# maxjiang93/space_time_pde

Measured on AMD Instinct MI355X. Metric: query-points/sec (fwd+PDE-residual bwd), rb2d 128^3 latent, higher is better.
Workload: dtype f32; 1 GPU; BASELINE configs[1]: latent [1,32,128,128,32], 2^20 query points, RB2 (3 transport + continuity), ImNet nf=32 softplus, L1 losses, backward to ImNet + UNet3d parameters; points=1048576, parallelism=points sharded x1, unet=UNet3d(igres=(32, 128, 128), nf=16, mf=256) fwd+bwd inside the timed step

## Files before the change

### include/stpde_hip.h

```cpp
#ifndef STPDE_HIP_H
#define STPDE_HIP_H

#ifdef __cplusplus
extern "C" {
#endif

#define STPDE_OK 0
#define STPDE_E_BADARG 1
#define STPDE_E_UNSUPPORTED 2
#define STPDE_E_LAUNCH 3

#define STPDE_ACT_TANH 0
#define STPDE_ACT_RELU 1
#define STPDE_ACT_SOFTPLUS 2
#define STPDE_ACT_ELU 3
#define STPDE_ACT_SWISH 4
#define STPDE_ACT_LEAKYRELU 5

#define STPDE_XT 3
#define STPDE_PBAR_SLOTS 64

typedef struct {
  int S1;
  int S2;
// ... 27 lines not shown
                     float* coef, int* cell, float* cw , void* stream);

typedef struct {
  int ntiles, KT, MT, first_hidden;
  stpde_jet_cfg cfg;
  int mfma_bf16;
  int packed;
  int det;
} stpde_layer_desc;
int stpde_jet_layer_fwd(const stpde_layer_desc* d, const float* in_pre, const float* X, const float* Wh_pack,
                        const float* Ws_pack, const float* tanc, const float* W0s_pack, const float* tanc0,
                        float* out_pre, const float* cw ,
                        const void* Wh_pack_bf16, float* z0, void* stream);

int stpde_jet_tail_fwd(const stpde_jet_cfg* cfg, int ntiles, int nf16, const float* in_pre2, const float* X,
                       const float* const* Wh_pack, const float* const* Ws_pack, const float* const* tanc,
                       float* const* out_pre, const float* cw, void* stream);

int stpde_jet_tail_fwd_p(const stpde_jet_cfg* cfg, int ntiles, int nf16, const float* in_pre2, const float* X,
                         const float* const* Wh_pack, const float* const* Ws_pack, const float* const* tanc,
                         float* const* out_pre, const float* cw, int packed, const void* const* Wh16_pack, void* stream);

int stpde_jet_tail_bwd(const stpde_jet_cfg* cfg, int ntiles, int nf16, const float* abar5, const float* const* WhT_pack,
                       const float* const* pre, float* const* abar_out, const float* cw, float* act_param_bar,
                       void* stream);

int stpde_jet_tail_bwd_p(const stpde_jet_cfg* cfg, int ntiles, int nf16, const float* abar5, const float* const* WhT_pack,
                         const float* const* pre, float* const* abar_out, const float* cw, float* act_param_bar, int packed,
                         const void* const* WhT16_pack, void* stream);

int stpde_jet_layer_bwd(const stpde_layer_desc* d, const float* abar_out, const float* WhT_pack, float* in_pre,
                        const float* X, const float* W0s_pack, const float* tanc0, float* abar0, const float* cw,
                        float* act_param_bar, const void* WhT_pack_bf16 ,
                        float* abar0_tan, const float* z0, void* stream);

int stpde_jet_layer_bwd_to(const stpde_layer_desc* d, const float* abar_out, const float* WhT_pack, const float* in_pre,
                           float* abar_in, const float* cw, float* act_param_bar, const void* WhT_pack_bf16, void* stream);

int stpde_jet_wgrad(const stpde_layer_desc* d, int SP, const float* abar_out, const float* in_pre, const float* X,
                    const float* tanc0, float* dW_aug, const float* cw, void* stream);

int stpde_jet_fc1_bwd_supported(const stpde_layer_desc* d);
int stpde_jet_fc1_bwd(const stpde_layer_desc* d, const float* abar1, const void* WhT_pack_bf16, const float* z0,
                      const float* tanc0, const float* cw, const float* X, float* abar0, float* abar0_tan, float* dW_aug,
                      float* act_param_bar, void* stream);

int stpde_lig_reduce_fwd(const stpde_jet_cfg* cfg, int S_mlp, int P, int n_out, const float* out_pre,
                         const float* coef, float* jets, long ldp, void* stream);
int stpde_lig_reduce_bwd(const stpde_jet_cfg* cfg, int S_mlp, int P, int n_out, const float* jets_bar, long ldp,
                         const float* coef, float* abar_out, void* stream);

int stpde_jet_tan0_reduce(int ntiles, int MT, const float* abar0_tan, float* dW_aug, int ldw, int det ,
                          void* stream);

typedef struct {
  int ntiles, nlayers, C, n1, n2;
  int MT[8];
  int SP[8];
  int packed[8];
  int S[8];
} stpde_xbar_desc;
int stpde_lig_xbar_scatter(const stpde_xbar_desc* d, const float* const* abar, const float* const* WsL_pack,
                           const int* cell, float* dlatent, void* stream);
int stpde_lig_xbar_rows(const stpde_xbar_desc* d, const float* const* abar, const float* const* WsL_pack,
                        float* xrows, void* stream);
int stpde_lig_dlatent_reduce(int B, int n0, int n1, int n2, int C, const float* xrows, const int* perm,
                             const int* start, float* dlatent, void* stream);

typedef struct {
  int nlayers;
  int cin, cout, nf16;
  int KT[8], MT[8];
  const float* Wh[8];
  const float* WhT[8];
  const float* Ws[8];
  const float* WsL[8];
  const float* tanc[8];
  const void* Wh16[8];
  const void* WhT16[8];
  int mfma_bf16;
  int packed_mask;
  long dw_off[8];
} stpde_imnet_plan;
typedef struct {
  float* X;
  float* XR;
  float* coef;
  float* cw;
  int* cell;
  float* pre[8];
  float* abar2x;
  float* abar3x;
  float* tan0;
  float* abar0;
  float* abar1x;
  float* abar0x;
  float* xrows;
  int* perm;
  int* start;
  void* sort_tmp;
  unsigned long sort_tmp_bytes;
  float* abar4x;
} stpde_lig_workspace;
#define STPDE_F_STASH 1
#define STPDE_F_VALUE_TILES 2
#define STPDE_F_FUSED_TAIL 4
// ... 246 lines not shown
```

### space_time_pde_amd/_lib.py

```python
import ctypes as C
import os
import subprocess
import threading

_HERE = os.path.dirname(os.path.abspath(__file__))
_CSRC = os.path.join(_HERE, "csrc")
LIB_PATH = os.environ.get("STPDE_LIB") or os.path.join(_HERE, "libstpde_hip.so")
_SOURCES = ["jet_layer.hip", "jet_layer_s00.hip", "jet_layer_s03.hip", "jet_layer_s30.hip", "jet_layer_s31.hip", "jet_layer_s32.hip", "jet_layer_s34.hip", "jet_layer_s36.hip", "jet_tail.hip", "jet_wgrad.hip", "jet_wgrad_s00.hip", "jet_wgrad_s30.hip", "jet_wgrad_s31.hip", "jet_wgrad_s32.hip", "jet_wgrad_s34.hip", "jet_wgrad_s36.hip", "jet_fc1_bwd.hip", "lig_gather_reduce.hip", "lig_pipeline.hip", "interp_nd.hip", "conv3d.hip", "conv3d_fused.hip", "optim.hip", "residual.hip", "bn.hip", "resample.hip", "sampler.hip", "sampler_median.hip", "api.cpp"]
_HIPFLAGS = ["--offload-arch=gfx950", "-O3", "-std=c++17", "-fPIC", "-ffp-contract=off", "-munsafe-fp-atomics",
             "--offload-compress"]

ABI_VERSION = 316

ACT_CODES = {"tanh": 0, "relu": 1, "softplus": 2, "elu": 3, "swish": 4, "leakyrelu": 5}
PBAR_SLOTS = 64
XT = 3


class JetCfg(C.Structure):
    _fields_ = [("S1", C.c_int), ("S2", C.c_int), ("pair0", C.c_int * 6), ("pair1", C.c_int * 6),
                ("act", C.c_int), ("act_param", C.c_float), ("combo", C.c_int), ("alpha", C.c_float * 6)]


class GatherDesc(C.Structure):
# ... 167 lines not shown
        objs.append(o)
        ostamp = o + ".srchash"
        owant = _source_hash([s] + _includes(s))
        if not force and os.path.exists(o) and os.path.exists(ostamp) and open(ostamp).read().strip() == owant:
            continue
        flags = _HIPFLAGS if s.endswith(".hip") else ["-O3", "-std=c++17", "-fPIC"]
        cmd = ["hipcc"] + flags + ["-c", s, "-o", o]
        if verbose:
            print(" ".join(cmd))
        procs.append((cmd, ostamp, owant, subprocess.Popen(cmd, stdout=subprocess.PIPE, stderr=subprocess.STDOUT)))
    for cmd, ostamp, owant, p in procs:
        out, _ = p.communicate()
        if p.returncode != 0:
            raise RuntimeError("hipcc failed: %s\n%s" % (" ".join(cmd), out.decode()))
        with open(ostamp, "w") as f:
            f.write(owant)
    cmd = ["hipcc", "--offload-arch=gfx950", "--offload-compress", "-shared", "-fPIC", "-o", LIB_PATH] + objs
    r = subprocess.run(cmd, stdout=subprocess.PIPE, stderr=subprocess.STDOUT)
    if r.returncode != 0:
        raise RuntimeError("link failed: %s\n%s" % (" ".join(cmd), r.stdout.decode()))
    with open(stamp, "w") as f:
        f.write(want)
    return LIB_PATH


_lib = None
_lock = threading.Lock()
_VP = C.c_void_p

_SIGNATURES = {
    "stpde_version": ([], C.c_int),
    "stpde_last_error": ([C.c_char_p, C.c_ulong], C.c_int),
    "stpde_tune": ([C.c_char_p, C.c_int], C.c_int),
    "stpde_trace_enable": ([C.c_int], C.c_int),
    "stpde_trace_read": ([C.c_char_p, C.c_ulong], C.c_long),
    "stpde_lig_gather": ([C.POINTER(GatherDesc), _VP, _VP, _VP, _VP, _VP, _VP, _VP, _VP], C.c_int),
    "stpde_lig_gather_nd": ([C.POINTER(GatherNdDesc), _VP, _VP, _VP, _VP, _VP], C.c_int),
    "stpde_lig_reduce_nd_fwd": ([C.c_int, C.c_int, C.c_int, C.c_int, _VP, _VP, _VP, C.c_long, _VP], C.c_int),
    "stpde_lig_reduce_nd_bwd": ([C.c_int, C.c_int, C.c_int, C.c_int, _VP, C.c_long, _VP, _VP, _VP], C.c_int),
    "stpde_lig_cell_nd": ([C.POINTER(GatherNdDesc), _VP, _VP, _VP], C.c_int),
    "stpde_lig_dlatent_reduce_nd": ([C.c_int, C.c_int, C.POINTER(C.c_int), C.c_int, _VP, _VP, _VP, _VP, _VP], C.c_int),
    "stpde_jet_layer_fwd": ([C.POINTER(LayerDesc)] + [_VP] * 12, C.c_int),
    "stpde_jet_layer_bwd": ([C.POINTER(LayerDesc)] + [_VP] * 13, C.c_int),
    "stpde_jet_layer_bwd_to": ([C.POINTER(LayerDesc)] + [_VP] * 8, C.c_int),
    "stpde_jet_tail_fwd": ([C.POINTER(JetCfg), C.c_int, C.c_int, _VP, _VP, C.POINTER(_VP), C.POINTER(_VP), C.POINTER(_VP),
                            C.POINTER(_VP), _VP, _VP], C.c_int),
    "stpde_jet_tail_bwd": ([C.POINTER(JetCfg), C.c_int, C.c_int, _VP, C.POINTER(_VP), C.POINTER(_VP), C.POINTER(_VP), _VP,
                            _VP, _VP], C.c_int),
    "stpde_jet_tail_fwd_p": ([C.POINTER(JetCfg), C.c_int, C.c_int, _VP, _VP, C.POINTER(_VP), C.POINTER(_VP), C.POINTER(_VP),
                              C.POINTER(_VP), _VP, C.c_int, C.POINTER(_VP), _VP], C.c_int),
    "stpde_jet_tail_bwd_p": ([C.POINTER(JetCfg), C.c_int, C.c_int, _VP, C.POINTER(_VP), C.POINTER(_VP), C.POINTER(_VP), _VP,
                              _VP, C.c_int, C.POINTER(_VP), _VP], C.c_int),
    "stpde_jet_tan0_reduce": ([C.c_int, C.c_int, _VP, _VP, C.c_int, C.c_int, _VP], C.c_int),
    "stpde_jet_wgrad": ([C.POINTER(LayerDesc), C.c_int] + [_VP] * 7, C.c_int),
    "stpde_jet_fc1_bwd_supported": ([C.POINTER(LayerDesc)], C.c_int),
    "stpde_jet_fc1_bwd": ([C.POINTER(LayerDesc)] + [_VP] * 11, C.c_int),
    "stpde_lig_reduce_fwd": ([C.POINTER(JetCfg), C.c_int, C.c_int, C.c_int, _VP, _VP, _VP, C.c_long, _VP], C.c_int),
    "stpde_lig_reduce_bwd": ([C.POINTER(JetCfg), C.c_int, C.c_int, C.c_int, _VP, C.c_long, _VP, _VP, _VP], C.c_int),
    "stpde_lig_xbar_scatter": ([C.POINTER(XbarDesc), C.POINTER(_VP), C.POINTER(_VP), _VP, _VP, _VP], C.c_int),
    "stpde_lig_xbar_rows": ([C.POINTER(XbarDesc), C.POINTER(_VP), C.POINTER(_VP), _VP, _VP], C.c_int),
    "stpde_lig_dlatent_reduce": ([C.c_int] * 5 + [_VP] * 5, C.c_int),
    "stpde_lig_imnet_jet_fwd": ([C.POINTER(ImNetPlanDesc), C.POINTER(JetCfg), C.POINTER(JetCfg), C.POINTER(GatherDesc), _VP,
                                 _VP, C.POINTER(LigWorkspace), _VP, C.c_long, C.c_int, _VP], C.c_int),
    "stpde_lig_imnet_jet_bwd": ([C.POINTER(ImNetPlanDesc), C.POINTER(JetCfg), C.POINTER(JetCfg), C.POINTER(JetCfg),
                                 C.POINTER(GatherDesc), C.POINTER(LigWorkspace), _VP, C.c_long, _VP, _VP, _VP, C.c_int, _VP],
                                C.c_int),
    "stpde_lig_sort_tmp_bytes": ([C.c_int, C.c_long], C.c_ulong),
    "stpde_lig_cell_sort": ([C.c_int, C.c_long, _VP, _VP, _VP, _VP, C.c_ulong, _VP], C.c_int),
    "stpde_interp_fwd": ([C.POINTER(InterpDesc)] + [_VP] * 7, C.c_int),
    "stpde_interp_bwd_grid": ([C.POINTER(InterpDesc)] + [_VP] * 5, C.c_int),
    "stpde_conv3d_fwd": ([C.POINTER(Conv3dDesc)] + [_VP] * 5, C.c_int),
    "stpde_conv3d_wgrad": ([C.POINTER(Conv3dDesc)] + [_VP] * 4, C.c_int),
    "stpde_conv3d_wgrad_bias": ([C.POINTER(Conv3dDesc)] + [_VP] * 5, C.c_int),
    "stpde_conv3d_fused": ([C.POINTER(Conv3dFusedArgs), C.POINTER(C.c_int), _VP], C.c_int),
    "stpde_conv3d_wgrad_onload": ([C.POINTER(Conv3dDesc)] + [_VP] * 8, C.c_int),
    "stpde_residual_fwd": ([_VP, C.c_int, C.c_int, C.c_int, C.c_int, _VP, C.c_long, C.c_long, _VP, _VP, _VP], C.c_int),
    "stpde_residual_bwd": ([_VP, C.c_int, C.c_int, C.c_int, C.c_int, _VP, C.c_long, C.c_long, _VP, _VP, _VP, _VP],
                           C.c_int),
    "stpde_resample3d": ([C.POINTER(ResampleDesc), C.c_int, _VP, _VP, _VP, _VP], C.c_int),
    "stpde_det_finalize": ([_VP, C.c_long, _VP, _VP], C.c_int),
    "stpde_bn_fwd": ([C.POINTER(BnDesc)] + [_VP] * 10, C.c_int),
    "stpde_bn_bwd": ([C.POINTER(BnDesc)] + [_VP] * 11, C.c_int),
    "stpde_loss_sum": ([C.c_int, C.c_long, _VP, _VP, _VP, _VP], C.c_int),
    "stpde_loss_grad": ([C.c_int, C.c_long, _VP, _VP, _VP, _VP, _VP], C.c_int),
    "stpde_clip_adam": ([C.POINTER(AdamDesc)] + [_VP] * 5, C.c_int),
    "stpde_clip_adam_multi": ([C.POINTER(AdamDesc), _VP, _VP, C.c_int, C.c_int, _VP], C.c_int),
    "stpde_opt_advance": ([C.POINTER(OptDesc), _VP, _VP], C.c_int),
    "stpde_clip_adam_dev": ([C.POINTER(AdamDesc)] + [_VP] * 6, C.c_int),
    "stpde_clip_adam_multi_dev": ([C.POINTER(AdamDesc), _VP, _VP, _VP, C.c_int, C.c_int, _VP], C.c_int),
    "stpde_clip_sgd": ([C.POINTER(SgdDesc)] + [_VP] * 5, C.c_int),
    "stpde_clip_sgd_multi": ([C.POINTER(SgdDesc), _VP, _VP, _VP, C.c_int, C.c_int, _VP], C.c_int),
    "stpde_sampler_draw": ([C.POINTER(SamplerDesc)] + [_VP] * 4, C.c_int),
    "stpde_sampler_produce": ([C.POINTER(SamplerDesc)] + [_VP] * 10, C.c_int),
    "stpde_sampler_filter": ([C.POINTER(SamplerFilterDesc)] + [_VP] * 9, C.c_int),
    "stpde_sampler_produce_filtered": ([C.POINTER(SamplerDesc)] + [_VP] * 8, C.c_int),
    "stpde_sampler_median": ([C.POINTER(SamplerFilterDesc)] + [_VP] * 5, C.c_int),
}


def exported_symbols():
    return sorted(_SIGNATURES)


def register_signatures(sigs):
    _SIGNATURES.update(sigs)

# ... 123 lines not shown
```

### space_time_pde_amd/csrc/common.h

```cpp
#pragma once
#include <hip/hip_runtime.h>

#include "../../include/stpde_hip.h"

typedef float f32x4 __attribute__((ext_vector_type(4)));

#define XT STPDE_XT
__host__ __device__ constexpr int x_live(int xt) { return xt == XT - 1 ? 1 : 4; }

__device__ __forceinline__ f32x4 ld4x(const float* p, int xt) {
  if (xt == XT - 1) return f32x4{p[0], 0.f, 0.f, 0.f};
  return *reinterpret_cast<const f32x4*>(p);
}

__device__ __forceinline__ f32x4 mfma4(float a, float b, f32x4 c) {
  return __builtin_amdgcn_mfma_f32_16x16x4f32(a, b, c, 0, 0, 0);
}

typedef __bf16 bf16x4 __attribute__((ext_vector_type(4)));
typedef __bf16 bf16x8 __attribute__((ext_vector_type(8)));
__device__ __forceinline__ bf16x4 to_bf4(f32x4 v) {
  bf16x4 r;
#pragma unroll
  for (int i = 0; i < 4; ++i) r[i] = (__bf16)v[i];
// ... 211 lines not shown
__device__ __forceinline__ f32x2 sel3(int d, f32x2 a0, f32x2 a1, f32x2 a2) { return d == 0 ? a0 : (d == 1 ? a1 : a2); }

template <int ACT>
__device__ __forceinline__ ActDT<f32x2> act_eval2_t(float prm, f32x2 a) {
  STPDE_JET_FMA
  ActDT<f32x2> r;
  if (ACT == STPDE_ACT_SOFTPLUS) {
    const f32x2 t = f32x2{-fabsf(a.x), -fabsf(a.y)} * 1.44269504088896341f;
    const f32x2 e = f32x2{__builtin_amdgcn_exp2f(t.x), __builtin_amdgcn_exp2f(t.y)};
    const f32x2 u = e + 1.f;
    const f32x2 inv = f32x2{fast_rcp(u.x), fast_rcp(u.y)};
    const f32x2 einv = e * inv;
    const f32x2 s = sel2(a.x >= 0.f, a.y >= 0.f, inv, einv);
    const f32x2 q = einv * inv;
    const bool b0 = a.x > 20.f, b1 = a.y > 20.f;
    const f32x2 lbig = f32x2{__builtin_amdgcn_logf(u.x), __builtin_amdgcn_logf(u.y)} * 0.693147180559945309f;
    const f32x2 lsmall = e * (1.f - e * (0.5f - e * 0.33333334f));
    const f32x2 l1p = sel2(e.x < 9.765625e-4f, e.y < 9.765625e-4f, lsmall, lbig);
    r.s0 = f32x2{fmaxf(a.x, 0.f), fmaxf(a.y, 0.f)} + l1p;
    const f32x2 one = f32x2{1.f, 1.f}, zero = f32x2{0.f, 0.f};
    r.s1 = sel2(b0, b1, one, s);
    r.s2 = sel2(b0, b1, zero, q);
    r.s3 = sel2(b0, b1, zero, q * (1.f - 2.f * s));
  } else {
    const ActD x = act_eval_t<ACT>(prm, a.x), y = act_eval_t<ACT>(prm, a.y);
    r.s0 = f32x2{x.s0, y.s0};
    r.s1 = f32x2{x.s1, y.s1};
    r.s2 = f32x2{x.s2, y.s2};
    r.s3 = f32x2{x.s3, y.s3};
  }
  return r;
}
template <int ACT>
__device__ __forceinline__ ActDT<f32x2> act_eval2(int act, float prm, f32x2 a) {
  if (ACT >= 0) return act_eval2_t<(ACT >= 0 ? ACT : 0)>(prm, a);
  const ActD x = act_eval<ACT>(act, prm, a.x), y = act_eval<ACT>(act, prm, a.y);
  ActDT<f32x2> r;
  r.s0 = f32x2{x.s0, y.s0};
  r.s1 = f32x2{x.s1, y.s1};
  r.s2 = f32x2{x.s2, y.s2};
  r.s3 = f32x2{x.s3, y.s3};
  return r;
}
template <int ACT>
__device__ __forceinline__ ActDT<float> act_eval_w(int act, float prm, float a) {
  const ActD s = act_eval<ACT>(act, prm, a);
  return ActDT<float>{s.s0, s.s1, s.s2, s.s3};
}
template <int ACT>
__device__ __forceinline__ ActDT<f32x2> act_eval_w(int act, float prm, f32x2 a) {
  return act_eval2<ACT>(act, prm, a);
}

template <int S1, int S2, int ACT, class T>
__device__ __forceinline__ void act_jet_fwd_w(const stpde_jet_cfg& cfg, const T* pre, T* h, const float* cq) {
  STPDE_JET_FMA
  const ActDT<T> s = act_eval_w<ACT>(cfg.act, cfg.act_param, pre[0]);
  h[0] = s.s0;
  if (S1 == 3) {
    const T a0 = pre[1], a1 = pre[2], a2 = pre[3];
    h[1] = s.s1 * a0;
    h[2] = s.s1 * a1;
    h[3] = s.s1 * a2;
    if (S2 == 1) {
      const T q = a0 * (cq[0] * a0 + cq[1] * a1 + cq[2] * a2) + a1 * (cq[3] * a1 + cq[4] * a2) + cq[5] * a2 * a2;
      h[4] = s.s2 * q + s.s1 * pre[4];
      return;
    }
#pragma unroll
    for (int p = 0; p < S2; ++p) {
      const T u = sel3(cfg.pair0[p], a0, a1, a2), v = sel3(cfg.pair1[p], a0, a1, a2);
      h[4 + p] = s.s2 * u * v + s.s1 * pre[4 + p];
    }
  }
}
template <int S1, int S2, int ACT>
__device__ __forceinline__ void act_jet_fwd(const stpde_jet_cfg& cfg, const f32x4* pre, f32x4* h,
                                            const float* cq = nullptr) {
  STPDE_JET_FMA
  constexpr int S = 1 + S1 + S2;
  if (S1 == 0 && S2 > 0) {
#pragma unroll
    for (int st = 0; st < 1 + S2; ++st) {
#if STPDE_JET_PACKED
      h[st].lo = act_eval_w<ACT>(cfg.act, cfg.act_param, (f32x2)pre[st].lo).s0;
      h[st].hi = act_eval_w<ACT>(cfg.act, cfg.act_param, (f32x2)pre[st].hi).s0;
#else
#pragma unroll
      for (int r = 0; r < 4; ++r) h[st][r] = act_eval<ACT>(cfg.act, cfg.act_param, pre[st][r]).s0;
#endif
    }
    return;
  }
#if STPDE_JET_PACKED
#pragma unroll
  for (int half = 0; half < 2; ++half) {
    f32x2 p2[S], h2[S];
#pragma unroll
    for (int st = 0; st < S; ++st) p2[st] = half ? (f32x2)pre[st].hi : (f32x2)pre[st].lo;
    act_jet_fwd_w<S1, S2, ACT, f32x2>(cfg, p2, h2, cq);
#pragma unroll
    for (int st = 0; st < S; ++st) {
      if (half) h[st].hi = h2[st];
      else h[st].lo = h2[st];
    }
  }
#else
#pragma unroll
  for (int r = 0; r < 4; ++r) {
    float p1[S], h1[S];
#pragma unroll
    for (int st = 0; st < S; ++st) p1[st] = pre[st][r];
    act_jet_fwd_w<S1, S2, ACT, float>(cfg, p1, h1, cq);
#pragma unroll
    for (int st = 0; st < S; ++st) h[st][r] = h1[st];
  }
#endif
}

template <int S1, int S2, int ACT, class T>
__device__ __forceinline__ void act_jet_adj_w(const stpde_jet_cfg& cfg, const T* pre, const T* hbar, T* abar, const float* cq) {
  STPDE_JET_FMA
  const ActDT<T> s = act_eval_w<ACT>(cfg.act, cfg.act_param, pre[0]);
  T ab = s.s1 * hbar[0];
  if (S1 == 3) {
    const T a0 = pre[1], a1 = pre[2], a2 = pre[3];
    T d0 = s.s1 * hbar[1], d1 = s.s1 * hbar[2], d2 = s.s1 * hbar[3];
    ab += s.s2 * (a0 * hbar[1] + a1 * hbar[2] + a2 * hbar[3]);
    if (S2 == 1) {
      const T hb = hbar[4];
      const T q = a0 * (cq[0] * a0 + cq[1] * a1 + cq[2] * a2) + a1 * (cq[3] * a1 + cq[4] * a2) + cq[5] * a2 * a2;
      ab += (s.s3 * q + s.s2 * pre[4]) * hb;
      const T t = s.s2 * hb;
      d0 += t * (2.f * cq[0] * a0 + cq[1] * a1 + cq[2] * a2);
      d1 += t * (cq[1] * a0 + 2.f * cq[3] * a1 + cq[4] * a2);
      d2 += t * (cq[2] * a0 + cq[4] * a1 + 2.f * cq[5] * a2);
      abar[4] = s.s1 * hb;
    }
#pragma unroll
    for (int p = 0; p < (S2 == 1 ? 0 : S2); ++p) {
      const int e0 = cfg.pair0[p], e1 = cfg.pair1[p];
      const T u = sel3(e0, a0, a1, a2), v = sel3(e1, a0, a1, a2);
      const T hb = hbar[4 + p];
      ab += (s.s3 * u * v + s.s2 * pre[4 + p]) * hb;
      const T t0 = s.s2 * v * hb;
      const T t1 = s.s2 * u * hb;
      const T z = t0 * 0.f;
      d0 += (e0 == 0 ? t0 : z) + (e1 == 0 ? t1 : z);
      d1 += (e0 == 1 ? t0 : z) + (e1 == 1 ? t1 : z);
      d2 += (e0 == 2 ? t0 : z) + (e1 == 2 ? t1 : z);
      abar[4 + p] = s.s1 * hb;
    }
    abar[1] = d0;
// ... 254 lines not shown
```

### space_time_pde_amd/csrc/jet_layer.hip

```cpp
#include "jet_layer_impl.h"

static int dispatch_streams(const LayerArgs& a, int mode, hipStream_t stream) {
  const int S1 = a.cfg.S1, S2 = a.cfg.S2;
  if (S1 == 0 && S2 == 0) return stpde_layer_launch_0_0(a, mode, stream);
  if (S1 == 0 && S2 == 3) return stpde_layer_launch_0_3(a, mode, stream);
  if (S1 == 3 && S2 == 0) return stpde_layer_launch_3_0(a, mode, stream);
  if (S1 == 3 && S2 == 1 && a.cfg.combo && a.cw) return stpde_layer_launch_3_1(a, mode, stream);
  if (S1 == 3 && S2 == 2) return stpde_layer_launch_3_2(a, mode, stream);
  if (S1 == 3 && S2 == 4) return stpde_layer_launch_3_4(a, mode, stream);
  if (S1 == 3 && S2 == 6) return stpde_layer_launch_3_6(a, mode, stream);
  stpde_set_error("stream configuration S1=%d S2=%d not compiled (supported: (0,0) (0,3 = four value tiles, forward only) (3,0) (3,1 combined, needs cw) (3,2) (3,4) (3,6))", S1, S2);
  return STPDE_E_UNSUPPORTED;
}

static int check_cfg(const stpde_layer_desc* d) {
  if (!d || d->ntiles <= 0 || d->MT <= 0 || d->KT < 0) {
    stpde_set_error("layer desc: bad sizes");
    return STPDE_E_BADARG;
  }
  if (d->cfg.act < 0 || d->cfg.act > 5) {
    stpde_set_error("layer desc: unknown activation %d", d->cfg.act);
    return STPDE_E_BADARG;
  }
  for (int p = 0; p < d->cfg.S2 && p < 6; ++p)
// ... 67 lines not shown
    return STPDE_E_BADARG;
  }
  return layer_bwd(d, abar_out, WhT_pack, in_pre, abar_in, nullptr, nullptr, nullptr, nullptr, cw, act_param_bar,
                   WhT_pack_bf16, nullptr, nullptr, stream);
}

static int layer_bwd(const stpde_layer_desc* d, const float* abar_out, const float* WhT_pack, const float* in_pre,
                     float* abar_in, const float* X, const float* W0s_pack, const float* tanc0, float* abar0,
                     const float* cw, float* act_param_bar, const void* WhT_pack_bf16, float* abar0_tan, const float* z0,
                     void* stream) {
  int rc = check_cfg(d);
  if (rc) return rc;
  LayerArgs a{};
  a.Bin = abar_out;
  a.Wp = WhT_pack;
  a.X = X;
  a.W0s = W0s_pack;
  a.tanc0 = tanc0;
  a.cw = cw;
  a.pbar = act_param_bar;
  a.Wp16 = d->mfma_bf16 ? WhT_pack_bf16 : nullptr;
  a.nsplit = d->mfma_bf16 == 3 ? 3 : 1;
  a.KT = d->MT;
  a.MT = d->KT;
  a.ntiles = d->ntiles;
  a.cfg = d->cfg;
  a.pk = ((d->packed & 4) ? 1 : 0) | ((d->packed & 2) ? 2 : 0) | ((d->packed & 1) ? 4 : 0);
  if (!abar_out || !WhT_pack || d->KT <= 0) {
    stpde_set_error("jet_layer_bwd: null pointer / no hidden input");
    return STPDE_E_BADARG;
  }
  if (d->first_hidden) {
    if (!z0 || !abar0 || (d->cfg.S1 && !tanc0)) {
      stpde_set_error("jet_layer_bwd: first_hidden needs z0/tanc0/abar0");
      return STPDE_E_BADARG;
    }
    if (z0 == abar0 && d->cfg.S1 && !abar0_tan) {
      stpde_set_error("jet_layer_bwd: z0 may alias abar0 only when abar0 holds the value stream alone");
      return STPDE_E_BADARG;
    }
    a.Out = abar0;
    a.Tan0 = abar0_tan;
    a.Z0 = const_cast<float*>(z0);
    return dispatch_streams(a, 3, (hipStream_t)stream);
  }
  if (!in_pre || !abar_in) {
    stpde_set_error("jet_layer_bwd: null in_pre");
    return STPDE_E_BADARG;
  }
  a.Out = abar_in;
  a.Pre = in_pre;
  return dispatch_streams(a, 2, (hipStream_t)stream);
}
```

### space_time_pde_amd/csrc/jet_layer_impl.h

```cpp
#pragma once
#include <cstdlib>

#include "common.h"

enum { PRO_NONE = 0, PRO_ACT = 1, PRO_L0 = 2 };
enum { EPI_FWD = 0, EPI_ADJ = 1, EPI_ADJ_L0 = 2 };
#ifndef STPDE_ABLATE
#define STPDE_ABLATE 0
#endif

#ifndef STPDE_STAMP
#define STPDE_STAMP 0
#endif
#ifndef STPDE_FWD2_OCC3
#define STPDE_FWD2_OCC3 1
#endif
#ifndef STPDE_FWD2_OCC_N
#define STPDE_FWD2_OCC_N 3
#endif
#ifndef STPDE_EARLY_L0
#define STPDE_EARLY_L0 1
#endif
#ifndef STPDE_EPI_PF
#define STPDE_EPI_PF 1
// ... 16 lines not shown
#ifndef STPDE_X3_Z0P
#define STPDE_X3_Z0P 0
#endif
#ifndef STPDE_SKIP_FIRST_BAR
#define STPDE_SKIP_FIRST_BAR 1
#endif
#if STPDE_STAMP
#define STPDE_STAMP_B0 8192
static __device__ unsigned long long g_stamp[256 * 8 * 16];
#define STAMP(i)                                                                                          \
  do {                                                                                                    \
    if (blockIdx.x >= STPDE_STAMP_B0 && blockIdx.x < STPDE_STAMP_B0 + 256 && (threadIdx.x & 63) == 0)     \
      g_stamp[((blockIdx.x - STPDE_STAMP_B0) * 8 + (threadIdx.x >> 6)) * 16 + (i)] = __builtin_readcyclecounter(); \
  } while (0)
#else
#define STAMP(i)
#endif

struct LayerArgs {
  const float* Bin;
  const float* Wp;
  const float* X;
  const float* W0s;
  const float* tanc0;
  const float* Wsp;
  const float* tanc;
  float* Out;
  const float* Pre;
  const float* cw;
  const void* Wp16;
  int nsplit;
  float* pbar;
  float* Tan0;
  float* Z0;
  int KT, MT, ntiles;
  int split;
  int pk;
  stpde_jet_cfg cfg;
};

__device__ __forceinline__ f32x4 layer0_block(const float* W0s, int nblk, int blk, int lo, const f32x4* xb) {
  f32x4 part[XT];
#pragma unroll
  for (int xt = 0; xt < XT; ++xt) {
    f32x4 w = ld4x(W0s + ((size_t)xt * nblk + blk) * 256 + lo, xt);
    f32x4 c = f32x4{0.f, 0.f, 0.f, 0.f};
#pragma unroll
    for (int r = 0; r < x_live(xt); ++r) c = mfma4(w[r], xb[xt][r], c);
    part[xt] = c;
  }
  return (part[0] + part[1]) + part[2];
}

template <int S1, int S2, int EPI, int ACT, int PKM = 0>
__device__ __forceinline__ void layer_epilogue(const LayerArgs& a, int tile, int mt, int MT, int lane, f32x4* accm,
                                               const f32x4 (*xbv)[XT], const float* cq, float& pacc,
                                               const f32x4* z0pre = nullptr, const f32x4* prepf = nullptr,
                                               const f32x4* wspf = nullptr, const f32x4* tcpf = nullptr) {
  constexpr int S = 1 + S1 + S2;
  constexpr bool VT = S1 == 0 && S2 > 0;
  const int lo = lane * 4;
  f32x4 (&acc)[1][S] = *reinterpret_cast<f32x4 (*)[1][S]>(accm);
  constexpr int mi = 0;
    if (EPI == EPI_FWD) {
#pragma unroll
      for (int xt = 0; xt < XT; ++xt) {
        f32x4 w = wspf ? wspf[xt] : ld4x(a.Wsp + ((size_t)xt * MT + mt) * 256 + lo, xt);
#pragma unroll
        for (int sv = 0; sv < (VT ? S : 1); ++sv)
#pragma unroll
          for (int r = 0; r < x_live(xt); ++r) acc[mi][sv] = mfma4(w[r], xbv[sv][xt][r], acc[mi][sv]);
      }
      if (S1 == 3) {
#pragma unroll
        for (int d = 0; d < 3; ++d) acc[mi][1 + d] += tcpf ? tcpf[d] : ld4(a.tanc + ((size_t)d * MT + mt) * 256 + lo);
      }
#pragma unroll
      for (int st = 0; st < S; ++st) st_blk(a.Out, (PKM & 2) ? 1 : 0, tile, S, MT, st, mt, lane, acc[mi][st]);
    } else {
      f32x4 pre[S], ab[S];
      if (EPI == EPI_ADJ) {
#pragma unroll
        for (int st = 0; st < S; ++st)
          pre[st] = prepf ? prepf[st] : ld_blk(a.Pre, (PKM & 4) ? 1 : 0, tile, S, MT, st, mt, lane);
      } else {
        pre[0] = z0pre ? *z0pre : ld4(a.Z0 + ((size_t)tile * MT + mt) * 256 + lo);
        if (S1 == 3) {
#pragma unroll
          for (int d = 0; d < 3; ++d) pre[1 + d] = tcpf ? tcpf[d] : ld4(a.tanc0 + ((size_t)d * MT + mt) * 256 + lo);
#pragma unroll
          for (int p = 0; p < S2; ++p) pre[4 + p] = f32x4{0.f, 0.f, 0.f, 0.f};
        }
      }
      act_jet_adj<S1, S2, ACT>(a.cfg, pre, acc[mi], ab, cq);
      if ((ACT == STPDE_ACT_SWISH || (ACT < 0 && a.cfg.act == STPDE_ACT_SWISH)) && a.pbar)
        pacc += swish_beta_adj<S1, S2>(a.cfg, pre, acc[mi], cq);
      constexpr int SO = (EPI == EPI_ADJ) ? S : 1 + S1;
      if (EPI == EPI_ADJ_L0 && S1 == 3 && a.Tan0) {
        st_blk(a.Out, (PKM & 2) ? 2 : 0, tile, 1, MT, 0, mt, lane, ab[0]);
        f32x4 ts[3];
#pragma unroll
        for (int d = 0; d < 3; ++d) ts[d] = row_sum16x4(ab[1 + d]);
        if ((lane & 15) == 15) {
          float* tp = a.Tan0 + ((size_t)tile * MT + mt) * 48 + 4 * (lane >> 4);
#pragma unroll
          for (int d = 0; d < 3; ++d) st4(tp + 16 * d, ts[d]);
        }
      } else {
#pragma unroll
        for (int st = 0; st < SO; ++st) st_blk(a.Out, (PKM & 2) ? 2 : 0, tile, SO, MT, st, mt, lane, ab[st]);
      }
    }
}

template <int EPI, int ACT>
__device__ __forceinline__ void flush_pbar(const LayerArgs& a, float pacc, int lane) {
  if (EPI != EPI_FWD && (ACT == STPDE_ACT_SWISH || (ACT < 0 && a.cfg.act == STPDE_ACT_SWISH)) && a.pbar) {
    const float v = wave_sum(pacc);
    if (lane == 0) atomicAdd(a.pbar + (blockIdx.x % STPDE_PBAR_SLOTS), v);
  }
}

template <int S1, int S2, int MC, int PRO, int EPI, int ACT, bool GUARD>
__global__ __launch_bounds__(256) void k_layer(LayerArgs a) {
  constexpr int S = 1 + S1 + S2;
  const int lane = threadIdx.x & 63;
  const int tile = blockIdx.x * 4 + (threadIdx.x >> 6);
  if (tile >= a.ntiles) return;
  const int KT = a.KT, MT = a.MT;
  const int lo = lane * 4;
  float cq[6];
  load_cq<S2>(a.cw, tile * 2 + ((lane & 15) >> 3), cq);
  float pacc = 0.f;

  constexpr bool VT = S1 == 0 && S2 > 0;
  constexpr int NX = VT ? S : 1;
  f32x4 xb[NX][XT];
  if (PRO == PRO_L0 || EPI == EPI_FWD) {
#pragma unroll
    for (int sv = 0; sv < NX; ++sv)
#pragma unroll
      for (int xt = 0; xt < XT; ++xt) xb[sv][xt] = ld4x(a.X + (((size_t)tile * NX + sv) * XT + xt) * 256 + lo, xt);
  }
  const auto z0r = opt_store_rsrc(a.Z0 ? a.Z0 + (size_t)tile * KT * 256 : nullptr, (unsigned)KT * 1024u);

  for (int mt0 = 0; mt0 < MT; mt0 += MC) {
  f32x4 acc[MC][S];
#pragma unroll
  for (int mi = 0; mi < MC; ++mi)
#pragma unroll
    for (int st = 0; st < S; ++st) acc[mi][st] = f32x4{0.f, 0.f, 0.f, 0.f};
  const float* wp = a.Wp + (size_t)mt0 * 256 + lo;

  auto load_raw = [&](int kt, f32x4* raw) {
    if (PRO == PRO_L0) {
#pragma unroll
      for (int sv = 0; sv < NX; ++sv) raw[sv] = layer0_block(a.W0s, KT, kt, lo, xb[sv]);
      if (!VT) opt_st4(z0r, kt * 1024 + lane * 16, raw[0]);
      if (S1 == 3) {
#pragma unroll
// ... 14 lines not shown
    }
  };

  if (KT > 0) {
    f32x4 Bc[S], wc[MC];
    {
      f32x4 raw[S];
      load_raw(0, raw);
      if (PRO == PRO_NONE) {
#pragma unroll
        for (int st = 0; st < S; ++st) Bc[st] = raw[st];
      } else {
        act_jet_fwd<S1, S2, ACT>(a.cfg, raw, Bc, cq);
      }
      load_w(0, wc);
    }
    for (int kt = 0; kt < KT; ++kt) {
      const int kn = kt + 1 < KT ? kt + 1 : kt;
      f32x4 rawn[S], wn[MC];
      load_raw(kn, rawn);
      load_w(kn, wn);
#pragma unroll
      for (int mi = 0; mi < MC; ++mi)
#pragma unroll
        for (int r = 0; r < 4; ++r)
#pragma unroll
          for (int st = 0; st < S; ++st) acc[mi][st] = mfma4(wc[mi][r], Bc[st][r], acc[mi][st]);
      if (PRO == PRO_NONE) {
#pragma unroll
        for (int st = 0; st < S; ++st) Bc[st] = rawn[st];
      } else {
        act_jet_fwd<S1, S2, ACT>(a.cfg, rawn, Bc, cq);
      }
#pragma unroll
      for (int mi = 0; mi < MC; ++mi) wc[mi] = wn[mi];
    }
  }

#pragma unroll
  for (int mi = 0; mi < MC; ++mi) {
    const int mt = mt0 + mi;
    if (GUARD && mt >= MT) continue;
    layer_epilogue<S1, S2, EPI, ACT>(a, tile, mt, MT, lane, acc[mi], xb, cq, pacc);
  }
  }
  flush_pbar<EPI, ACT>(a, pacc, lane);
}


template <int S1, int S2, int MCg, int PRO, int EPI, int ACT, int NW, bool BF = false, int PK = 1, bool WRING = false,
          int SPL = 1, int PKM = 0>
__global__ __launch_bounds__(64 * NW, ((!BF || SPL == 1) && PRO == PRO_ACT && EPI == EPI_FWD && MCg == 2 && NW == 4 && !WRING && S1 + S2 <= 4 && STPDE_FWD2_OCC3) ? STPDE_FWD2_OCC_N : 2) void k_layer_coop(LayerArgs a) {
  constexpr int S = 1 + S1 + S2, GK = NW * PK;
  static_assert(!WRING || (!BF && GK == 4), "the weight ring is written for 4 k-tiles per group, fp32");
  static_assert(SPL == 1 || (BF && SPL == 3), "operand splitting is a bf16-pipe mode");
  constexpr int BMODE = (PKM & 1) ? (EPI == EPI_FWD ? 1 : 2) : 0;
  __shared__ __attribute__((aligned(16))) float hb[2][GK][S][BF ? 128 * SPL : 256];
  const int lane = threadIdx.x & 63;
  const int wv = threadIdx.x >> 6;
  const int KT = a.KT, MT = a.MT;
  const int lo = lane * 4;
  STAMP(0);
  int tile = blockIdx.x, pass0 = 0, pstep = 1;
  if (a.split > 0) {
    const int L = blockIdx.x, xcd = L & 7, slot = L >> 3;
    pass0 = slot % a.split;
    pstep = a.split;
    tile = (slot / a.split) * 8 + xcd;
    if (tile >= a.ntiles) return;
  }
  float cq[6];
  load_cq<S2>(a.cw, tile * 2 + ((lane & 15) >> 3), cq);
  float pacc = 0.f;

  constexpr bool VT = S1 == 0 && S2 > 0;
  constexpr int NX = VT ? S : 1;
  f32x4 xb[NX][XT];
  if (PRO == PRO_L0 || EPI == EPI_FWD) {
#pragma unroll
    for (int sv = 0; sv < NX; ++sv)
#pragma unroll
      for (int xt = 0; xt < XT; ++xt) xb[sv][xt] = ld4x(a.X + (((size_t)tile * NX + sv) * XT + xt) * 256 + lo, xt);
  }
  const auto z0r = opt_store_rsrc(a.Z0 ? a.Z0 + (size_t)tile * KT * 256 : nullptr, (unsigned)KT * 1024u);

  auto produce = [&](int kt, int buf, int slot) {
    f32x4 raw[S], B[S];
    if (PRO == PRO_L0) {
#pragma unroll
      for (int sv = 0; sv < NX; ++sv) raw[sv] = layer0_block(a.W0s, KT, kt, lo, xb[sv]);
      if (!VT) opt_st4(z0r, kt * 1024 + lane * 16, raw[0]);
      if (S1 == 3) {
#pragma unroll
        for (int d = 0; d < 3; ++d) raw[1 + d] = ld4(a.tanc0 + ((size_t)d * KT + kt) * 256 + lo);
#pragma unroll
        for (int p = 0; p < S2; ++p) raw[4 + p] = f32x4{0.f, 0.f, 0.f, 0.f};
      }
    } else {
#pragma unroll
      for (int st = 0; st < S; ++st) raw[st] = ld_blk(a.Bin, BMODE, tile, S, KT, st, kt, lane);
    }
    if (PRO == PRO_NONE || STPDE_ABLATE == 1) {
#pragma unroll
      for (int st = 0; st < S; ++st) B[st] = raw[st];
    } else {
      act_jet_fwd<S1, S2, ACT>(a.cfg, raw, B, cq);
    }
#pragma unroll
    for (int st = 0; st < S; ++st) {
      if constexpr (BF) {
        f32x4 v = B[st];
#pragma unroll
        for (int t = 0; t < SPL; ++t) {
          const bf16x4 h = to_bf4(v);
          *reinterpret_cast<bf16x4*>(&hb[buf][slot][st][128 * t + lane * 2]) = h;
          if (t + 1 < SPL) v -= bf4_to_f32(h);
        }
      } else {
        st4(&hb[buf][slot][st][lo], B[st]);
      }
    }
  };
  auto store_block = [&](const f32x4* B, int buf, int slot) {
#pragma unroll
    for (int st = 0; st < S; ++st) {
      if constexpr (BF) {
        f32x4 v = B[st];
#pragma unroll
        for (int t = 0; t < SPL; ++t) {
          const bf16x4 h = to_bf4(v);
          *reinterpret_cast<bf16x4*>(&hb[buf][slot][st][128 * t + lane * 2]) = h;
          if (t + 1 < SPL) v -= bf4_to_f32(h);
        }
      } else {
        st4(&hb[buf][slot][st][lo], B[st]);
      }
    }
  };
  auto produce_group = [&](int g, int buf) {
#pragma unroll
    for (int k = 0; k < PK; ++k) produce(GK * g + NW * k + wv, buf, NW * k + wv);
  };

  const int ngroups = KT / GK;
  bool first_pass = true;
  for (int mt0 = (pass0 * NW + wv) * MCg; mt0 < MT; mt0 += pstep * NW * MCg) {
    f32x4 acc[MCg][S];
#pragma unroll
    for (int mi = 0; mi < MCg; ++mi)
#pragma unroll
      for (int st = 0; st < S; ++st) acc[mi][st] = f32x4{0.f, 0.f, 0.f, 0.f};
    constexpr bool Z0P = EPI == EPI_ADJ_L0 && (SPL == 1 || STPDE_X3_Z0P);
    f32x4 z0p[Z0P ? MCg : 1];
    if constexpr (Z0P) {
#pragma unroll
      for (int mi = 0; mi < MCg; ++mi) z0p[mi] = ld4(a.Z0 + ((size_t)tile * MT + mt0 + mi) * 256 + lo);
    }
    const float* wp = a.Wp + (size_t)mt0 * 256 + lo;
    f32x4 wr[WRING ? 4 : 1][MCg];
    if constexpr (WRING) {
#pragma unroll
      for (int q = 0; q < 3; ++q)
#pragma unroll
        for (int mi = 0; mi < MCg; ++mi) wr[q][mi] = ld4(wp + ((size_t)q * MT + mi) * 256);
    }
    if (!STPDE_SKIP_FIRST_BAR || !first_pass) __syncthreads();
    first_pass = false;
    STAMP(1);
    produce_group(0, 0);
    STAMP(2);
    __syncthreads();
    STAMP(3);
    for (int gi = 0; gi < ngroups; ++gi) {
      const int buf = gi & 1;
      const int gnext = gi + 1 < ngroups ? gi + 1 : gi;
      constexpr bool EARLY = PRO == PRO_NONE && (SPL == 1 || STPDE_X3_EARLY);
      constexpr bool EARLY0 = PRO == PRO_L0 && !VT && STPDE_EARLY_L0;
      f32x4 rawn[EARLY ? PK : 1][S];
      if constexpr (EARLY) {
#pragma unroll
        for (int k = 0; k < PK; ++k)
#pragma unroll
          for (int st = 0; st < S; ++st)
            rawn[k][st] = ld_blk(a.Bin, BMODE, tile, S, KT, st, GK * gnext + NW * k + wv, lane);
      }
      f32x4 w0n[EARLY0 ? PK : 1][XT], tcn[EARLY0 ? PK : 1][3];
      if constexpr (EARLY0) {
#pragma unroll
        for (int k = 0; k < PK; ++k) {
          const int kt = GK * gnext + NW * k + wv;
#pragma unroll
          for (int xt = 0; xt < XT; ++xt) w0n[k][xt] = ld4x(a.W0s + ((size_t)xt * KT + kt) * 256 + lo, xt);
          if (S1 == 3) {
#pragma unroll
            for (int d = 0; d < 3; ++d) tcn[k][d] = ld4(a.tanc0 + ((size_t)d * KT + kt) * 256 + lo);
          }
        }
// ... 72 lines not shown
          const int ktn = STPDE_ABLATE == 3 ? (q & 1) : (kt + 3 < KT ? kt + 3 : KT - 1);
          f32x4 B[S];
#pragma unroll
          for (int st = 0; st < S; ++st) B[st] = ld4(&hb[buf][q][st][lo]);
#pragma unroll
          for (int mi = 0; mi < MCg; ++mi)
#pragma unroll
            for (int r = 0; r < 4; ++r)
#pragma unroll
              for (int st = 0; st < S; ++st) acc[mi][st] = mfma4(wr[q][mi][r], B[st][r], acc[mi][st]);
#pragma unroll
          for (int mi = 0; mi < MCg; ++mi) wr[(q + 3) & 3][mi] = ld4(wp + ((size_t)ktn * MT + mi) * 256);
        }
      } else {
#pragma unroll
      for (int q = 0; q < GK; ++q) {
        const int kt = GK * gi + q;
        f32x4 B[S], w[MCg];
#pragma unroll
        for (int st = 0; st < S; ++st) B[st] = ld4(&hb[buf][q][st][lo]);
#pragma unroll
        for (int mi = 0; mi < MCg; ++mi) w[mi] = ld4(wp + ((size_t)kt * MT + mi) * 256);
#pragma unroll
        for (int mi = 0; mi < MCg; ++mi)
#pragma unroll
          for (int r = 0; r < 4; ++r)
#pragma unroll
            for (int st = 0; st < S; ++st) acc[mi][st] = mfma4(w[mi][r], B[st][r], acc[mi][st]);
      }
      }
      if constexpr (EARLY) {
#pragma unroll
        for (int k = 0; k < PK; ++k) store_block(rawn[k], buf ^ 1, NW * k + wv);
      } else if constexpr (EARLY0) {
#pragma unroll
        for (int k = 0; k < PK; ++k) {
          const int kt = GK * gnext + NW * k + wv;
          f32x4 raw[S], B[S], part[XT];
#pragma unroll
          for (int xt = 0; xt < XT; ++xt) {
            f32x4 c = f32x4{0.f, 0.f, 0.f, 0.f};
#pragma unroll
            for (int r = 0; r < x_live(xt); ++r) c = mfma4(w0n[k][xt][r], xb[0][xt][r], c);
            part[xt] = c;
          }
          raw[0] = (part[0] + part[1]) + part[2];
          opt_st4(z0r, kt * 1024 + lane * 16, raw[0]);
          if (S1 == 3) {
#pragma unroll
            for (int d = 0; d < 3; ++d) raw[1 + d] = tcn[k][d];
#pragma unroll
            for (int p = 0; p < S2; ++p) raw[4 + p] = f32x4{0.f, 0.f, 0.f, 0.f};
          }
          act_jet_fwd<S1, S2, ACT>(a.cfg, raw, B, cq);
          store_block(B, buf ^ 1, NW * k + wv);
        }
      } else {
        if (STPDE_ABLATE != 5) produce_group(gnext, buf ^ 1);
      }
      if (gi < 8) STAMP(4 + gi);
      if (STPDE_ABLATE != 2) __syncthreads();
    }
    STAMP(12);
    if (STPDE_ABLATE == 4) {
      f32x4 sum = f32x4{0.f, 0.f, 0.f, 0.f};
#pragma unroll
      for (int mi = 0; mi < MCg; ++mi)
#pragma unroll
        for (int st = 0; st < S; ++st) sum += acc[mi][st];
      if (sum[0] == 12345.678f) st4(a.Out + lo, sum);
      continue;
    }
    constexpr bool EPF = EPI == EPI_ADJ && (!BF || (SPL == 1 && STPDE_EPI_PF_BF)) && MCg > 1 && STPDE_EPI_PF;
    if constexpr (EPF) {
      constexpr int PMD = (PKM & 4) ? 1 : 0;
      constexpr int PFD = STPDE_EPI_PF_DEPTH < 1 ? 1 : (STPDE_EPI_PF_DEPTH > MCg ? MCg : STPDE_EPI_PF_DEPTH);
      f32x4 pr[MCg][S];
#pragma unroll
      for (int mi = 0; mi < PFD; ++mi)
#pragma unroll
        for (int st = 0; st < S; ++st) pr[mi][st] = ld_blk(a.Pre, PMD, tile, S, MT, st, mt0 + mi, lane);
#pragma unroll
      for (int mi = 0; mi < MCg; ++mi) {
        if (mi + PFD < MCg) {
#pragma unroll
          for (int st = 0; st < S; ++st) pr[mi + PFD][st] = ld_blk(a.Pre, PMD, tile, S, MT, st, mt0 + mi + PFD, lane);
        }
        __builtin_amdgcn_sched_barrier(0);
        layer_epilogue<S1, S2, EPI, ACT, PKM>(a, tile, mt0 + mi, MT, lane, acc[mi], xb, cq, pacc, nullptr, pr[mi]);
      }
    } else if constexpr (EPI == EPI_ADJ_L0 && S1 == 3 && S <= 5 && (STPDE_EPI_OPF & 1) && (SPL == 1 || (STPDE_EPI_OPF & 4))) {
      if constexpr (SPL == 1) {
        f32x4 z0l[MCg], tcl[MCg][3];
#pragma unroll
        for (int mi = 0; mi < MCg; ++mi) {
          z0l[mi] = Z0P ? z0p[Z0P ? mi : 0] : ld4(a.Z0 + ((size_t)tile * MT + mt0 + mi) * 256 + lo);
#pragma unroll
          for (int d = 0; d < 3; ++d) tcl[mi][d] = ld4(a.tanc0 + ((size_t)d * MT + mt0 + mi) * 256 + lo);
        }
        __builtin_amdgcn_sched_barrier(0);
#pragma unroll
        for (int mi = 0; mi < MCg; ++mi)
          layer_epilogue<S1, S2, EPI, ACT, PKM>(a, tile, mt0 + mi, MT, lane, acc[mi], xb, cq, pacc, &z0l[mi], nullptr, nullptr,
                                                  tcl[mi]);
      } else {
        f32x4 zc, zn, tcc[3], tcn2[3];
        auto fetch = [&](int mt, f32x4& z, f32x4* t) {
// ... 189 lines not shown
```

Before: 2.497 million query-points/s.

## Use packed-FP32 jet quadratic, DPP row-sum fold, and scalar wave index

```diff
diff --git a/include/stpde_hip.h b/include/stpde_hip.h
--- a/include/stpde_hip.h
+++ b/include/stpde_hip.h
@@ -103,6 +103,8 @@
 
 int stpde_jet_tan0_reduce(int ntiles, int MT, const float* abar0_tan, float* dW_aug, int ldw, int det ,
                           void* stream);
+
+int stpde_jet_rowsum_probe(int ntiles, const float* in, float* out, void* stream);
 
 typedef struct {
   int ntiles, nlayers, C, n1, n2;
diff --git a/space_time_pde_amd/_lib.py b/space_time_pde_amd/_lib.py
--- a/space_time_pde_amd/_lib.py
+++ b/space_time_pde_amd/_lib.py
@@ -243,6 +243,7 @@
     "stpde_jet_tail_bwd_p": ([C.POINTER(JetCfg), C.c_int, C.c_int, _VP, C.POINTER(_VP), C.POINTER(_VP), C.POINTER(_VP), _VP,
                               _VP, C.c_int, C.POINTER(_VP), _VP], C.c_int),
     "stpde_jet_tan0_reduce": ([C.c_int, C.c_int, _VP, _VP, C.c_int, C.c_int, _VP], C.c_int),
+    "stpde_jet_rowsum_probe": ([C.c_int, _VP, _VP, _VP], C.c_int),
     "stpde_jet_wgrad": ([C.POINTER(LayerDesc), C.c_int] + [_VP] * 7, C.c_int),
     "stpde_jet_fc1_bwd_supported": ([C.POINTER(LayerDesc)], C.c_int),
     "stpde_jet_fc1_bwd": ([C.POINTER(LayerDesc)] + [_VP] * 11, C.c_int),
diff --git a/space_time_pde_amd/csrc/common.h b/space_time_pde_amd/csrc/common.h
--- a/space_time_pde_amd/csrc/common.h
+++ b/space_time_pde_amd/csrc/common.h
@@ -287,7 +287,34 @@
   return act_eval2<ACT>(act, prm, a);
 }
 
-template <int S1, int S2, int ACT, class T>
+__device__ __forceinline__ f32x2 pk_mul(f32x2 a, f32x2 b) {
+  f32x2 r;
+  asm("v_pk_mul_f32 %0, %1, %2" : "=v"(r) : "v"(a), "v"(b));
+  return r;
+}
+__device__ __forceinline__ f32x2 pk_fma(f32x2 a, f32x2 b, f32x2 c) {
+  f32x2 r;
+  asm("v_pk_fma_f32 %0, %1, %2, %3" : "=v"(r) : "v"(a), "v"(b), "v"(c));
+  return r;
+}
+
+template <bool W, class T>
+__device__ __forceinline__ T jet_q(T a0, T a1, T a2, const float* cq) {
+  STPDE_JET_FMA
+  return a0 * (cq[0] * a0 + cq[1] * a1 + cq[2] * a2) + a1 * (cq[3] * a1 + cq[4] * a2) + cq[5] * a2 * a2;
+}
+template <>
+__device__ __forceinline__ f32x2 jet_q<true, f32x2>(f32x2 a0, f32x2 a1, f32x2 a2, const float* cq) {
+  const f32x2 c0 = f32x2{cq[0], cq[0]}, c1 = f32x2{cq[1], cq[1]}, c2 = f32x2{cq[2], cq[2]};
+  const f32x2 c3 = f32x2{cq[3], cq[3]}, c4 = f32x2{cq[4], cq[4]}, c5 = f32x2{cq[5], cq[5]};
+  f32x2 i0 = pk_fma(c0, a0, pk_mul(c1, a1));
+  const f32x2 i1 = pk_fma(c3, a1, pk_mul(c4, a2));
+  i0 = pk_fma(c2, a2, i0);
+  const f32x2 q = pk_fma(a0, i0, pk_mul(a1, i1));
+  return pk_fma(a2, pk_mul(c5, a2), q);
+}
+
+template <int S1, int S2, int ACT, class T, bool W = false>
 __device__ __forceinline__ void act_jet_fwd_w(const stpde_jet_cfg& cfg, const T* pre, T* h, const float* cq) {
   STPDE_JET_FMA
   const ActDT<T> s = act_eval_w<ACT>(cfg.act, cfg.act_param, pre[0]);
@@ -298,7 +325,7 @@
     h[2] = s.s1 * a1;
     h[3] = s.s1 * a2;
     if (S2 == 1) {
-      const T q = a0 * (cq[0] * a0 + cq[1] * a1 + cq[2] * a2) + a1 * (cq[3] * a1 + cq[4] * a2) + cq[5] * a2 * a2;
+      const T q = jet_q<W, T>(a0, a1, a2, cq);
       h[4] = s.s2 * q + s.s1 * pre[4];
       return;
     }
@@ -309,7 +336,7 @@
     }
   }
 }
-template <int S1, int S2, int ACT>
+template <int S1, int S2, int ACT, bool W = false>
 __device__ __forceinline__ void act_jet_fwd(const stpde_jet_cfg& cfg, const f32x4* pre, f32x4* h,
                                             const float* cq = nullptr) {
   STPDE_JET_FMA
@@ -333,7 +360,7 @@
     f32x2 p2[S], h2[S];
 #pragma unroll
     for (int st = 0; st < S; ++st) p2[st] = half ? (f32x2)pre[st].hi : (f32x2)pre[st].lo;
-    act_jet_fwd_w<S1, S2, ACT, f32x2>(cfg, p2, h2, cq);
+    act_jet_fwd_w<S1, S2, ACT, f32x2, W>(cfg, p2, h2, cq);
 #pragma unroll
     for (int st = 0; st < S; ++st) {
       if (half) h[st].hi = h2[st];
diff --git a/space_time_pde_amd/csrc/jet_layer.hip b/space_time_pde_amd/csrc/jet_layer.hip
--- a/space_time_pde_amd/csrc/jet_layer.hip
+++ b/space_time_pde_amd/csrc/jet_layer.hip
@@ -143,3 +143,24 @@
   a.Pre = in_pre;
   return dispatch_streams(a, 2, (hipStream_t)stream);
 }
+
+__global__ __launch_bounds__(256) void k_rowsum_probe(const float* in, float* out, int ntiles) {
+  const int lane = threadIdx.x & 63;
+  const int tile = blockIdx.x * 4 + (threadIdx.x >> 6);
+  if (tile >= ntiles) return;
+  f32x4 v[3];
+#pragma unroll
+  for (int d = 0; d < 3; ++d)
+#pragma unroll
+    for (int j = 0; j < 4; ++j) v[d][j] = in[((size_t)tile * 12 + 4 * d + j) * 64 + lane];
+  store_tan_rowsums(out + (size_t)tile * 48, lane, v);
+}
+
+extern "C" int stpde_jet_rowsum_probe(int ntiles, const float* in, float* out, void* stream) {
+  if (ntiles <= 0 || !in || !out) {
+    stpde_set_error("jet_rowsum_probe: bad arguments");
+    return STPDE_E_BADARG;
+  }
+  STPDE_LAUNCH(k_rowsum_probe, dim3((ntiles + 3) / 4), dim3(256), 0, (hipStream_t)stream, in, out, ntiles);
+  return stpde_check_launch("k_rowsum_probe");
+}
diff --git a/space_time_pde_amd/csrc/jet_layer_impl.h b/space_time_pde_amd/csrc/jet_layer_impl.h
--- a/space_time_pde_amd/csrc/jet_layer_impl.h
+++ b/space_time_pde_amd/csrc/jet_layer_impl.h
@@ -92,6 +92,62 @@
   return (part[0] + part[1]) + part[2];
 }
 
+__device__ __forceinline__ void row_sum16_fold12(const f32x4* v, float* e) {
+  float r0 = v[0][0], r1 = v[0][1], r2 = v[0][2], r3 = v[0][3], r4 = v[1][0], r5 = v[1][1], r6 = v[1][2], r7 = v[1][3];
+  float r8 = v[2][0], r9 = v[2][1], r10 = v[2][2], r11 = v[2][3], t0, t1, t2;
+  const unsigned long long even = 0x5555555555555555ull, low2 = 0x3333333333333333ull;
+  asm volatile(
+      "s_nop 1\n\t"
+      "v_cndmask_b32_e64 %12, %1, %0, %15\n\t"
+      "v_cndmask_b32_e64 %13, %3, %2, %15\n\t"
+      "v_cndmask_b32_e64 %14, %5, %4, %15\n\t"
+      "v_cndmask_b32_e64 %0, %0, %1, %15\n\t"
+      "v_cndmask_b32_e64 %2, %2, %3, %15\n\t"
+      "v_cndmask_b32_e64 %4, %4, %5, %15\n\t"
+      "v_add_f32_dpp %1, %0, %12 quad_perm:[1,0,3,2] row_mask:0xf bank_mask:0xf\n\t"
+      "v_add_f32_dpp %3, %2, %13 quad_perm:[1,0,3,2] row_mask:0xf bank_mask:0xf\n\t"
+      "v_add_f32_dpp %5, %4, %14 quad_perm:[1,0,3,2] row_mask:0xf bank_mask:0xf\n\t"
+      "v_cndmask_b32_e64 %12, %7, %6, %15\n\t"
+      "v_cndmask_b32_e64 %13, %9, %8, %15\n\t"
+      "v_cndmask_b32_e64 %14, %11, %10, %15\n\t"
+      "v_cndmask_b32_e64 %6, %6, %7, %15\n\t"
+      "v_cndmask_b32_e64 %8, %8, %9, %15\n\t"
+      "v_cndmask_b32_e64 %10, %10, %11, %15\n\t"
+      "v_add_f32_dpp %7, %6, %12 quad_perm:[1,0,3,2] row_mask:0xf bank_mask:0xf\n\t"
+      "v_add_f32_dpp %9, %8, %13 quad_perm:[1,0,3,2] row_mask:0xf bank_mask:0xf\n\t"
+      "v_add_f32_dpp %11, %10, %14 quad_perm:[1,0,3,2] row_mask:0xf bank_mask:0xf\n\t"
+      "v_cndmask_b32_e64 %12, %3, %1, %16\n\t"
+      "v_cndmask_b32_e64 %13, %7, %5, %16\n\t"
+      "v_cndmask_b32_e64 %14, %11, %9, %16\n\t"
+      "v_cndmask_b32_e64 %1, %1, %3, %16\n\t"
+      "v_cndmask_b32_e64 %5, %5, %7, %16\n\t"
+      "v_cndmask_b32_e64 %9, %9, %11, %16\n\t"
+      "v_add_f32_dpp %3, %1, %12 quad_perm:[2,3,0,1] row_mask:0xf bank_mask:0xf\n\t"
+      "v_add_f32_dpp %7, %5, %13 quad_perm:[2,3,0,1] row_mask:0xf bank_mask:0xf\n\t"
+      "v_add_f32_dpp %11, %9, %14 quad_perm:[2,3,0,1] row_mask:0xf bank_mask:0xf\n\t"
+      "v_add_f32_dpp %3, %3, %3 row_shr:4 row_mask:0xf bank_mask:0xf bound_ctrl:1\n\t"
+      "v_add_f32_dpp %7, %7, %7 row_shr:4 row_mask:0xf bank_mask:0xf bound_ctrl:1\n\t"
+      "v_add_f32_dpp %11, %11, %11 row_shr:4 row_mask:0xf bank_mask:0xf bound_ctrl:1\n\t"
+      "v_add_f32_dpp %3, %3, %3 row_shr:8 row_mask:0xf bank_mask:0xf bound_ctrl:1\n\t"
+      "v_add_f32_dpp %7, %7, %7 row_shr:8 row_mask:0xf bank_mask:0xf bound_ctrl:1\n\t"
+      "v_add_f32_dpp %11, %11, %11 row_shr:8 row_mask:0xf bank_mask:0xf bound_ctrl:1"
+      : "+v"(r0), "+v"(r1), "+v"(r2), "+v"(r3), "+v"(r4), "+v"(r5), "+v"(r6), "+v"(r7), "+v"(r8), "+v"(r9), "+v"(r10),
+        "+v"(r11), "=&v"(t0), "=&v"(t1), "=&v"(t2)
+      : "s"(even), "s"(low2));
+  e[0] = r3;
+  e[1] = r7;
+  e[2] = r11;
+}
+__device__ __forceinline__ void store_tan_rowsums(float* tan, int lane, const f32x4* ab_tan) {
+  float e[3];
+  row_sum16_fold12(ab_tan, e);
+  if ((lane & 15) >= 12) {
+    float* tp = tan + 4 * (lane >> 4) + (lane & 3);
+#pragma unroll
+    for (int d = 0; d < 3; ++d) tp[16 * d] = e[d];
+  }
+}
+
 template <int S1, int S2, int EPI, int ACT, int PKM = 0>
 __device__ __forceinline__ void layer_epilogue(const LayerArgs& a, int tile, int mt, int MT, int lane, f32x4* accm,
                                                const f32x4 (*xbv)[XT], const float* cq, float& pacc,
@@ -138,14 +194,7 @@
       constexpr int SO = (EPI == EPI_ADJ) ? S : 1 + S1;
       if (EPI == EPI_ADJ_L0 && S1 == 3 && a.Tan0) {
         st_blk(a.Out, (PKM & 2) ? 2 : 0, tile, 1, MT, 0, mt, lane, ab[0]);
-        f32x4 ts[3];
-#pragma unroll
-        for (int d = 0; d < 3; ++d) ts[d] = row_sum16x4(ab[1 + d]);
-        if ((lane & 15) == 15) {
-          float* tp = a.Tan0 + ((size_t)tile * MT + mt) * 48 + 4 * (lane >> 4);
-#pragma unroll
-          for (int d = 0; d < 3; ++d) st4(tp + 16 * d, ts[d]);
-        }
+        store_tan_rowsums(a.Tan0 + ((size_t)tile * MT + mt) * 48, lane, ab + 1);
       } else {
 #pragma unroll
         for (int st = 0; st < SO; ++st) st_blk(a.Out, (PKM & 2) ? 2 : 0, tile, SO, MT, st, mt, lane, ab[st]);
@@ -266,12 +315,13 @@
           int SPL = 1, int PKM = 0>
 __global__ __launch_bounds__(64 * NW, ((!BF || SPL == 1) && PRO == PRO_ACT && EPI == EPI_FWD && MCg == 2 && NW == 4 && !WRING && S1 + S2 <= 4 && STPDE_FWD2_OCC3) ? STPDE_FWD2_OCC_N : 2) void k_layer_coop(LayerArgs a) {
   constexpr int S = 1 + S1 + S2, GK = NW * PK;
+  constexpr bool WH = !BF;
   static_assert(!WRING || (!BF && GK == 4), "the weight ring is written for 4 k-tiles per group, fp32");
   static_assert(SPL == 1 || (BF && SPL == 3), "operand splitting is a bf16-pipe mode");
   constexpr int BMODE = (PKM & 1) ? (EPI == EPI_FWD ? 1 : 2) : 0;
   __shared__ __attribute__((aligned(16))) float hb[2][GK][S][BF ? 128 * SPL : 256];
   const int lane = threadIdx.x & 63;
-  const int wv = threadIdx.x >> 6;
+  const int wv = __builtin_amdgcn_readfirstlane(threadIdx.x >> 6);
   const int KT = a.KT, MT = a.MT;
   const int lo = lane * 4;
   STAMP(0);
@@ -318,7 +368,7 @@
 #pragma unroll
       for (int st = 0; st < S; ++st) B[st] = raw[st];
     } else {
-      act_jet_fwd<S1, S2, ACT>(a.cfg, raw, B, cq);
+      act_jet_fwd<S1, S2, ACT, WH>(a.cfg, raw, B, cq);
     }
 #pragma unroll
     for (int st = 0; st < S; ++st) {
@@ -357,6 +407,7 @@
   };
 
   const int ngroups = KT / GK;
+  __builtin_assume(ngroups >= 1);
   bool first_pass = true;
   for (int mt0 = (pass0 * NW + wv) * MCg; mt0 < MT; mt0 += pstep * NW * MCg) {
     f32x4 acc[MCg][S];
@@ -535,7 +586,7 @@
 #pragma unroll
             for (int p = 0; p < S2; ++p) raw[4 + p] = f32x4{0.f, 0.f, 0.f, 0.f};
           }
-          act_jet_fwd<S1, S2, ACT>(a.cfg, raw, B, cq);
+          act_jet_fwd<S1, S2, ACT, WH>(a.cfg, raw, B, cq);
           store_block(B, buf ^ 1, NW * k + wv);
         }
       } else {
```

Measured after the change: 2.519 million query-points/s (median of 6 runs). About the same (+0.9%).
